# sp-uhh/audio-visual-vad

Measured on AMD Instinct MI355X. Metric: AV frame-pairs/sec (fwd+bwd), higher is better.
Workload: dtype f32; 1 GPU; AV_net fused training step (WaveNet-W0 encoder + ResNet-18 trunk + concat + 2xLSTM1024 + FC, masked BCE, backward, RCCL all-reduce, fused Adam): BASELINE configs[3]/[4] per-GPU shard; per_gpu_frame_pairs=1024, global_frame_pairs=1024, sequences_per_gpu=64, parallelism=dp1, reserved_cus=0, reported_block=median

## Files before the change

audio-visual-vad_amd/csrc/igemm.h:

```cpp
#pragma once
#include "common.h"
#include <type_traits>

namespace igemm {

constexpr int BK = 32;

struct NoCtx {};

struct EpiStore {
  static constexpr bool PLAIN = true;
  float* C;
  long ldc;
  const float* bias;
  int mode;
  int cs = 1;
  double* stat = nullptr;
  __device__ __forceinline__ float* ptr(int m, int n) const { return C + (long)m * ldc + (long)n * cs; }
};
template <class Epi, class = void>
struct HasStat : std::false_type {};
template <class Epi>
struct HasStat<Epi, std::void_t<decltype(Epi::stat)>> : std::true_type {};

// ... 255 lines not shown
  int X, K, relu;
  __device__ __forceinline__ Ctx prep(int) const { return Ctx(); }
  __device__ __forceinline__ typename std::conditional<BUF, void, bool>::type load(const Ctx&, int x, int k0, int kin, float* v) const {
    const int k = k0 + kin;
    const bool ok = k < K && x < X;
    if constexpr (BUF) {
      static_assert(V == 4, "buffer form: 16-byte fetches");
      const f4v t = bload4(brsrc2g(p), ok ? (int)(((unsigned)k * (unsigned)ld + (unsigned)x) * 4u) : BUF_OOB, 0);
      v[0] = t[0]; v[1] = t[1]; v[2] = t[2]; v[3] = t[3];
    } else {
      const long off = ok ? (long)k * ld + x : 0;
      if (V == 4) {
        const float4 t = *reinterpret_cast<const float4*>(p + off);
        v[0] = t.x; v[1] = t.y; v[2] = t.z; v[3] = t.w;
      } else {
        v[0] = p[off];
      }
      return ok;
    }
  }
  __device__ __forceinline__ float post(float v) const { return relu ? fmaxf(v, 0.f) : v; }
};

#ifdef AVVAD_PROF
__device__ unsigned long long g_prof[8];
__device__ unsigned long long g_prof_blk[2 * 2048];
__device__ unsigned long long g_prof_clk[2048];
__device__ unsigned long long g_prof_hw[2048];
#define PROF_T() ((wave == 0) ? __builtin_amdgcn_s_memtime() : 0ull)
#define PROF_ADD(i, v) do { if (t == 0) atomicAdd(&g_prof[i], (unsigned long long)(v)); } while (0)
#else
#define PROF_T() 0ull
#define PROF_ADD(i, v) do { } while (0)
#endif

template <class Op, class = void>
struct HasPost : std::false_type {};
template <class Op>
struct HasPost<Op, std::void_t<decltype(&Op::post)>> : std::true_type {};

template <class Op, class = void>
struct HasPrep2 : std::false_type {};
template <class Op>
struct HasPrep2<Op, std::void_t<decltype(&Op::prep2)>> : std::true_type {};
template <class Op, class = void>
struct PerVec : std::false_type {};
template <class Op>
struct PerVec<Op, std::void_t<decltype(Op::PERVEC)>> : std::integral_constant<bool, Op::PERVEC> {};

template <class Epi, class = void>
struct IsPlain : std::false_type {};
template <class Epi>
struct IsPlain<Epi, std::void_t<decltype(Epi::PLAIN)>> : std::integral_constant<bool, Epi::PLAIN> {};
template <class Epi, class = void>
struct HasFinish : std::false_type {};
template <class Epi>
struct HasFinish<Epi, std::void_t<decltype(&Epi::finish4)>> : std::true_type {};

typedef __bf16 bf16x8 __attribute__((ext_vector_type(8)));
typedef __bf16 bf16x4 __attribute__((ext_vector_type(4)));
typedef float f32x4v __attribute__((ext_vector_type(4)));
constexpr int LDH = 40;

template <class Op, int BX, int NTH>
struct Stage {
  static constexpr int VEC = Op::VEC;
  static constexpr int NV = BX * BK / (NTH * VEC);
  static constexpr int LD = Op::KCONTIG ? BX + 1 : BX + 4;
  static constexpr int NCTX = (Op::KCONTIG || PerVec<Op>::value) ? NV : 1;
  static constexpr int TILE_F32 = BK * LD;
  static constexpr int TILE_BF = BX * LDH / 2;
  __device__ static __forceinline__ void coord(int t, int i, int& xl, int& kl) {
    if (Op::KCONTIG) {
      if (VEC == 4) { kl = (t & 7) * 4; xl = (t >> 3) + (NTH / 8) * i; }
      else { kl = t & 31; xl = (t >> 5) + (NTH / 32) * i; }
    } else {
      if (VEC == 4) { constexpr int Q = BX / 4; xl = (t % Q) * 4; kl = t / Q + (NTH / Q) * i; }
      else { xl = t % BX; kl = t / BX + (NTH / BX) * i; }
    }
  }
  __device__ static __forceinline__ void to_lds(float* S, int t, const float (&st0)[NV][VEC], const Op& op, unsigned okmask) {
    float st[NV][VEC];
#pragma unroll
    for (int i = 0; i < NV; ++i)
#pragma unroll
      for (int j = 0; j < VEC; ++j) {
        float v = st0[i][j];
        if constexpr (HasPost<Op>::value) v = op.post(v);
#ifdef AVVAD_ABL_NOSEL
        st[i][j] = v;
#else
        st[i][j] = ((okmask >> i) & 1u) ? v : 0.f;
#endif
      }
#pragma unroll
    for (int i = 0; i < NV; ++i) {
      int xl, kl;
      coord(t, i, xl, kl);
      if constexpr (Op::KCONTIG) {
#pragma unroll
        for (int j = 0; j < VEC; ++j) S[(kl + j) * LD + xl] = st[i][j];
      } else if constexpr (VEC == 4) {
        *reinterpret_cast<float4*>(S + kl * LD + xl) = make_float4(st[i][0], st[i][1], st[i][2], st[i][3]);
      } else {
        S[kl * LD + xl] = st[i][0];
      }
    }
  }
  __device__ static __forceinline__ void to_lds_bf(__bf16* S, int t, const float (&st0)[NV][VEC], const Op& op, unsigned okmask) {
#pragma unroll
    for (int i = 0; i < NV; ++i) {
// ... 338 lines not shown
#pragma unroll
              for (int r = 0; r < 16; ++r) old[r] = Cb[base + (unsigned)mfma32_row(r, 0) * ld32];
#pragma unroll
              for (int r = 0; r < 16; ++r) Cb[base + (unsigned)mfma32_row(r, 0) * ld32] = old[r] + acc[i][j][r] + bv;
            }
            continue;
          }
        }
#pragma unroll
        for (int r = 0; r < 16; ++r) {
          const int m = mb + mfma32_row(r, lh_e);
          if (m < Mv && n < N) {
            float* p;
            if constexpr (HasSched<Epi>::value) p = Cv + (long)m * E.ldc + n;
            else p = E.ptr(m, n);
            const float v = acc[i][j][r] + bv;
            if (atomic) atomicAdd(p, v);
            else if (E.mode == 0) *p = v;
            else *p += v;
          }
        }
      }
#ifdef AVVAD_PROF
    const unsigned long long tp3 = PROF_T();
    PROF_ADD(0, 1); PROF_ADD(1, tp1 - tp0); PROF_ADD(2, tp2 - tp1); PROF_ADD(3, tbar); PROF_ADD(4, tstage); PROF_ADD(5, tp3 - tp2);
    PROF_ADD(6, kt1 - kt0);
#endif
  }
#ifdef AVVAD_PROF
  if (t == 0 && blockIdx.x < 2048) {
    g_prof_blk[2 * blockIdx.x + 1] = __builtin_amdgcn_s_memrealtime();
    g_prof_clk[blockIdx.x] = __builtin_amdgcn_s_memtime() - g_prof_clk[blockIdx.x];
  }
#endif
}

template <int BM, int BN, class Epi>
__global__ void __launch_bounds__(256)
    fixup(const Epi E, const float* __restrict__ slab, const int M, const int N, const int ktiles, const long G,
          const int full_rounds, const int rem_tiles, const int ntn) {
  constexpr int STRIPS = BM * BN / 256;
  __shared__ float4 part[3][64];
  const int tr = blockIdx.x / STRIPS, strip = blockIdx.x % STRIPS;
  unsigned R = (unsigned)rem_tiles * (unsigned)ktiles, it0 = (unsigned)tr * (unsigned)ktiles, it1 = it0 + (unsigned)ktiles - 1u;
  const unsigned Gu = (unsigned)G;
  if constexpr (HasSched<Epi>::value) {
    R = (unsigned)E.sched.total();
    it0 = (unsigned)E.sched.base(tr);
    it1 = it0 + (unsigned)E.sched.len(tr) - 1u;
  }
  const int ga = (int)(((it0 + 1u) * Gu + R - 1u) / R) - 1, gb = (int)(((it1 + 1u) * Gu + R - 1u) / R) - 1;
  const int lane = threadIdx.x & 63, wave = threadIdx.x >> 6;
  const int e0 = strip * 256 + lane * 4;
  if (gb <= ga) {
    if constexpr (HasFinish<Epi>::value) {
      if (E.active && wave == 0) {
        const unsigned tile_u = (unsigned)full_rounds * Gu + (unsigned)tr;
        const int mu = (int)(tile_u / (unsigned)ntn) * BM + e0 / BN, nu = (int)(tile_u % (unsigned)ntn) * BN + e0 % BN;
        if (epi_live(E, mu, M)) {
          float v[4] = {0.f, 0.f, 0.f, 0.f};
#pragma unroll
          for (int e = 0; e < 4; ++e)
            if (nu + e < N) v[e] = *E.ptr(mu, nu + e);
          E.finish4(mu, nu, v, N);
        }
      }
    }
    return;
  }
  const bool sparse = R < Gu;
  const float* S0 = slab + e0;
  float4 sum = make_float4(0.f, 0.f, 0.f, 0.f);
  for (int g = ga + 1 + wave; g <= gb; g += 16) {
    float4 v[4];
    bool ok[4];
#pragma unroll
    for (int u = 0; u < 4; ++u) {
      const int gu = g + 4 * u;
      ok[u] = gu <= gb && (!sparse || ((unsigned)(gu + 1) * R) / Gu > ((unsigned)gu * R) / Gu);
      v[u] = *reinterpret_cast<const float4*>(S0 + (long)(ok[u] ? gu : ga + 1) * (BM * BN));
    }
#pragma unroll
    for (int u = 0; u < 4; ++u)
      if (ok[u]) { sum.x += v[u].x; sum.y += v[u].y; sum.z += v[u].z; sum.w += v[u].w; }
  }
  if (wave > 0) part[wave - 1][lane] = sum;
  __syncthreads();
  if (wave > 0) return;
#pragma unroll
  for (int w = 0; w < 3; ++w) { const float4 p = part[w][lane]; sum.x += p.x; sum.y += p.y; sum.z += p.z; sum.w += p.w; }
  const unsigned tile = (unsigned)full_rounds * Gu + (unsigned)tr;
  const int m = (int)(tile / (unsigned)ntn) * BM + e0 / BN, n0 = (int)(tile % (unsigned)ntn) * BN + e0 % BN;
  if (!epi_live(E, m, M)) return;
  const float sv[4] = {sum.x, sum.y, sum.z, sum.w};
  if constexpr (HasFinish<Epi>::value) {
    if (E.active) {
      float v[4] = {0.f, 0.f, 0.f, 0.f};
#pragma unroll
      for (int e = 0; e < 4; ++e)
        if (n0 + e < N) v[e] = *E.ptr(m, n0 + e) + sv[e];
      E.finish4(m, n0, v, N);
      return;
    }
  }
#pragma unroll
  for (int e = 0; e < 4; ++e)
    if (n0 + e < N) *E.ptr(m, n0 + e) += sv[e];
}

template <int BM, int BN, class Epi>
__global__ void __launch_bounds__(256)
    fixup1(const Epi E, const float* __restrict__ slab, const int M, const int N, const int ktiles, const long G,
           const int full_rounds, const int rem_tiles, const int ntn) {
  constexpr int STRIPS = BM * BN / 256;
  const int lane = threadIdx.x & 63, wave = threadIdx.x >> 6;
  const int sg = blockIdx.x * 4 + wave;
  const int tr = sg / STRIPS, strip = sg % STRIPS;
  if (tr >= rem_tiles) return;
  unsigned R = (unsigned)rem_tiles * (unsigned)ktiles, it0 = (unsigned)tr * (unsigned)ktiles, it1 = it0 + (unsigned)ktiles - 1u;
  const unsigned Gu = (unsigned)G;
  if constexpr (HasSched<Epi>::value) {
    R = (unsigned)E.sched.total();
    it0 = (unsigned)E.sched.base(tr);
    it1 = it0 + (unsigned)E.sched.len(tr) - 1u;
  }
  const int ga = (int)(((it0 + 1u) * Gu + R - 1u) / R) - 1, gb = (int)(((it1 + 1u) * Gu + R - 1u) / R) - 1;
  const int e0 = strip * 256 + lane * 4;
  const unsigned tile = (unsigned)full_rounds * Gu + (unsigned)tr;
  const int m = (int)(tile / (unsigned)ntn) * BM + e0 / BN, n0 = (int)(tile % (unsigned)ntn) * BN + e0 % BN;
  if (!epi_live(E, m, M)) return;
  float4 sum = make_float4(0.f, 0.f, 0.f, 0.f);
  if (gb > ga) {
    const bool sparse = R < Gu;
    const float* S0 = slab + e0;
    for (int g = ga + 1; g <= gb; g += 4) {
      float4 v[4];
      bool ok[4];
#pragma unroll
      for (int u = 0; u < 4; ++u) {
        const int gu = g + u;
        ok[u] = gu <= gb && (!sparse || ((unsigned)(gu + 1) * R) / Gu > ((unsigned)gu * R) / Gu);
        v[u] = *reinterpret_cast<const float4*>(S0 + (long)(ok[u] ? gu : ga + 1) * (BM * BN));
      }
#pragma unroll
      for (int u = 0; u < 4; ++u)
        if (ok[u]) { sum.x += v[u].x; sum.y += v[u].y; sum.z += v[u].z; sum.w += v[u].w; }
    }
  } else if (!HasFinish<Epi>::value) {
    return;
  }
  const float sv[4] = {sum.x, sum.y, sum.z, sum.w};
  if constexpr (HasFinish<Epi>::value) {
    if (E.active) {
      float v[4] = {0.f, 0.f, 0.f, 0.f};
#pragma unroll
      for (int e = 0; e < 4; ++e)
        if (n0 + e < N) v[e] = *E.ptr(m, n0 + e) + sv[e];
      E.finish4(m, n0, v, N);
      return;
    }
    if (gb <= ga) return;
  }
#pragma unroll
  for (int e = 0; e < 4; ++e)
    if (n0 + e < N) *E.ptr(m, n0 + e) += sv[e];
}

template <int BM, int BN, class Epi = EpiStore>
__global__ void __launch_bounds__(256)
    fixup_tile(const Epi E, const float* __restrict__ slab, const int M, const int N, const int ktiles, const long G,
               const int full_rounds, const int rem_tiles, const int ntn) {
  constexpr int CQ = BN / 4, RG = 256 / CQ, RPT = BM / RG;
  static_assert(RPT % 4 == 0, "four rows in flight per thread");
  __shared__ double red[RG * BN * 2];
  const int tr = blockIdx.x;
  unsigned R = (unsigned)rem_tiles * (unsigned)ktiles, it0 = (unsigned)tr * (unsigned)ktiles, it1 = it0 + (unsigned)ktiles - 1u;
  const unsigned Gu = (unsigned)G;
  if constexpr (HasSched<Epi>::value) {
    R = (unsigned)E.sched.total();
    it0 = (unsigned)E.sched.base(tr);
    it1 = it0 + (unsigned)E.sched.len(tr) - 1u;
  }
  const int ga = (int)(((it0 + 1u) * Gu + R - 1u) / R) - 1, gb = (int)(((it1 + 1u) * Gu + R - 1u) / R) - 1;
  if (gb <= ga) return;
  const bool sparse = R < Gu;
  const unsigned tile = (unsigned)full_rounds * Gu + (unsigned)tr;
  const int tm = (int)(tile / (unsigned)ntn);
  const int m0 = tm * BM, n0 = (int)(tile % (unsigned)ntn) * BN;
  float* Cv = E.C;
  int mrow0 = m0, Mv = M;
  if constexpr (HasSched<Epi>::value) { const auto v = E.view(m0); Cv = v.C; mrow0 = v.row0; Mv = v.M; }
  const int cq = threadIdx.x % CQ, rg = threadIdx.x / CQ;
  const int n = n0 + cq * 4;
  float s4[4] = {0.f, 0.f, 0.f, 0.f}, q4[4] = {0.f, 0.f, 0.f, 0.f};
  if (n < N) {
#pragma unroll 1
    for (int rr = 0; rr < RPT; rr += 4) {
      float4 tot[4];
      bool live[4];
      const float* sp[4];
#pragma unroll
      for (int u = 0; u < 4; ++u) {
        const int row = rg + RG * (rr + u);
        live[u] = mrow0 + row < Mv;
        sp[u] = slab + (long)(live[u] ? row : 0) * BN + cq * 4;
        tot[u] = make_float4(0.f, 0.f, 0.f, 0.f);
      }
      for (int g = ga + 1; g <= gb; ++g) {
        if (sparse && !(((unsigned)(g + 1) * R) / Gu > ((unsigned)g * R) / Gu)) continue;
        float4 v[4];
#pragma unroll
        for (int u = 0; u < 4; ++u) v[u] = *reinterpret_cast<const float4*>(sp[u] + (long)g * (BM * BN));
#pragma unroll
        for (int u = 0; u < 4; ++u) { tot[u].x += v[u].x; tot[u].y += v[u].y; tot[u].z += v[u].z; tot[u].w += v[u].w; }
      }
#pragma unroll
      for (int u = 0; u < 4; ++u) {
        if (!live[u]) continue;
        float4* const cp = reinterpret_cast<float4*>(Cv + (long)(mrow0 + rg + RG * (rr + u)) * E.ldc + n);
        float4 o = *cp;
        o.x += tot[u].x; o.y += tot[u].y; o.z += tot[u].z; o.w += tot[u].w;
        *cp = o;
        s4[0] += o.x; s4[1] += o.y; s4[2] += o.z; s4[3] += o.w;
        q4[0] = fmaf(o.x, o.x, q4[0]); q4[1] = fmaf(o.y, o.y, q4[1]); q4[2] = fmaf(o.z, o.z, q4[2]); q4[3] = fmaf(o.w, o.w, q4[3]);
      }
    }
  }
  if (E.stat == nullptr) return;
#pragma unroll
  for (int e = 0; e < 4; ++e) {
    red[(rg * BN + cq * 4 + e) * 2 + 0] = (double)s4[e];
    red[(rg * BN + cq * 4 + e) * 2 + 1] = (double)q4[e];
  }
  __syncthreads();
  const int c = threadIdx.x;
  if (c < BN && n0 + c < N) {
    double a = 0, b = 0;
#pragma unroll 4
    for (int w = 0; w < RG; ++w) { a += red[(w * BN + c) * 2 + 0]; b += red[(w * BN + c) * 2 + 1]; }
    E.stat[((long)tm * 2 + 0) * N + n0 + c] = a;
    E.stat[((long)tm * 2 + 1) * N + n0 + c] = b;
  }
}

constexpr int NUM_CU = 256;

constexpr size_t SLAB_FLOATS = (size_t)256 * 576 * 64;
static_assert(SLAB_FLOATS >= (size_t)512 * 128 * 128, "one 128x128 tile per persistent worker");

template <int BM, int BN, class AOp, class BOp, class Epi>
static inline int launch(const AOp& a, const BOp& b, const Epi& e_in, int M, int N, int K, int split_k_hint,
                         hipStream_t s, float* slab = nullptr, bool allow_bf16 = true, bool* finished = nullptr) {
  Epi e = e_in;
  if (M <= 0 || N <= 0 || K <= 0) return AVVAD_EINVAL;
  const int ktiles = (K + BK - 1) / BK;
  const long ntiles = (long)cdiv(M, BM) * cdiv(N, BN);
  const long iters = ntiles * ktiles;
  const AvvadTune& tn = avvad_tune();
  const int var = tn.igemm_variant;
  constexpr bool BIG = (BM == 128 && BN == 128);
  constexpr bool TALL = (BM == 256);
  const int variant = TALL ? 3 : (var >= 0 ? var : (BIG ? 2 : 1));
  int per_cu;
  if (variant == 3) per_cu = 2;
  else if (variant == 0) per_cu = BIG ? 2 : (BM * BN >= 128 * 64 ? 3 : 4);
  else if (variant == 1 || !BIG) per_cu = BIG ? 3 : (BM * BN >= 128 * 64 ? 4 : 6);
  else per_cu = 2;
  const int cus = (tn.max_cus > 0 && tn.max_cus < NUM_CU) ? tn.max_cus : NUM_CU;
  long G = (long)cus * per_cu;
  if (G * BM * BN > (long)SLAB_FLOATS) G = (long)(SLAB_FLOATS / ((size_t)BM * BN));
  const bool no_sk = !slab || tn.no_streamk == 1 || tn.no_streamk == 10 + e.mode ||
                     (double)ntiles * ktiles * (double)G >= 4.0e9;
  long full_rounds = ntiles / G, rem = ntiles - full_rounds * G;
  int kchunks = 0;
  if (split_k_hint > 1 && e.mode != 0 && ntiles <= G && tn.kmajor) {
    long best = -1;
    for (int r = 1; r <= 2; ++r) {
      long nc = r * G / ntiles;
      if (nc > ktiles) nc = ktiles;
      if (nc < 1) nc = 1;
      const long rr = (nc * ntiles + G - 1) / G;
      const long cost = rr * ((ktiles + nc - 1) / nc) + rr * 8;
      if (best < 0 || cost < best) { best = cost; kchunks = (int)nc; }
    }
    full_rounds = 0; rem = 0;
    if ((long)kchunks * ntiles < G) G = (long)kchunks * ntiles;
  } else {
    if (no_sk || rem * 10 >= G * 9) {
      if (rem > 0) ++full_rounds;
      rem = 0;
    }
    if (rem > 0 && full_rounds == 0) {
      const long cap = iters / 4 > 0 ? iters / 4 : 1;
      if (G > cap) G = cap;
    }
  }
  const int fr = (int)full_rounds, rt = (int)rem;
  const bool bf = allow_bf16 && tn.bf16;
  bool stat = false;
  if constexpr (std::is_same<Epi, EpiStore>::value) {
    stat = e.stat != nullptr;
    if (stat && (e.cs != 1 || (e.ldc & 3) || (N & 3) || (((uintptr_t)e.C) & 15) || kchunks > 0 || e.bias != nullptr)) return AVVAD_EINVAL;
  }
  if constexpr (HasFinish<Epi>::value) {
    e.active = (rt > 0 && kchunks == 0 && fr == 0 && (long)rt == ntiles) ? 1 : 0;
    if (finished) *finished = e.active != 0;
  } else if (finished) {
    *finished = false;
  }
  const int kflags = tn.stagger ? 1 : 0;
#define AVVAD_IGEMM_LAUNCH(DBV, NTHV)                                                                                       \
  do {                                                                                                                      \
    if (bf)                                                                                                                 \
      hipLaunchKernelGGL((kernel<BM, BN, DBV, NTHV, AOp, BOp, Epi, true>), dim3((int)G), dim3(NTHV), 0, s, a, b, e, M, N, kflags, \
                         ktiles, fr, rt, kchunks, slab);                                                                    \
    else                                                                                                                    \
      hipLaunchKernelGGL((kernel<BM, BN, DBV, NTHV, AOp, BOp, Epi, false>), dim3((int)G), dim3(NTHV), 0, s, a, b, e, M, N, kflags, \
                         ktiles, fr, rt, kchunks, slab);                                                                    \
  } while (0)
  if constexpr (TALL) {
    AVVAD_IGEMM_LAUNCH(false, 512);
  } else {
    if (variant == 0) AVVAD_IGEMM_LAUNCH(true, 256);
    else if (variant == 1 || !BIG) AVVAD_IGEMM_LAUNCH(false, 256);
    else AVVAD_IGEMM_LAUNCH(true, (BIG ? 512 : 256));
  }
#undef AVVAD_IGEMM_LAUNCH
  if (rt > 0 && kchunks == 0 && stat) {
    if constexpr (std::is_same<Epi, EpiStore>::value)
      hipLaunchKernelGGL((fixup_tile<BM, BN>), dim3(rt), dim3(256), 0, s, e, slab, M, N, ktiles, G, fr, rt, cdiv(N, BN));
  } else if (rt > 0 && kchunks == 0) {
    const int deep = tn.no_fixup1 > 1 ? tn.no_fixup1 : 6;
    if ((G + rt - 1) / rt <= deep && tn.no_fixup1 != 1)
      hipLaunchKernelGGL((fixup1<BM, BN, Epi>), dim3(rt * (BM * BN / 1024)), dim3(256), 0, s, e, slab, M, N, ktiles, G, fr, rt, cdiv(N, BN));
    else
      hipLaunchKernelGGL((fixup<BM, BN, Epi>), dim3(rt * (BM * BN / 256)), dim3(256), 0, s, e, slab, M, N, ktiles, G, fr, rt, cdiv(N, BN));
  }
  AVVAD_LAUNCH_CHECK();
  return AVVAD_OK;
}

template <class AOp, class BOp, class Epi>
static inline int launch_cls(const AOp& a, const BOp& b, const Epi& e, int Mp, int N, hipStream_t s, float* slab) {
  constexpr int BM = 128, BN = 128;
  if (Mp <= 0 || N <= 0 || !slab) return AVVAD_EINVAL;
  const AvvadTune& tn = avvad_tune();
  const long ntiles = (long)cdiv(Mp, BM) * cdiv(N, BN);
  const int cus = (tn.max_cus > 0 && tn.max_cus < NUM_CU) ? tn.max_cus : NUM_CU;
  long G = (long)cus * 2;
  if (G * BM * BN > (long)SLAB_FLOATS) G = (long)(SLAB_FLOATS / ((size_t)BM * BN));
  const long R = e.sched.total();
  if (R <= 0 || (double)R * (double)G >= 4.0e9) return AVVAD_EINVAL;
  if (G > R / 4) G = R / 4 > 0 ? R / 4 : 1;
  bool stat = false;
  if constexpr (HasStat<Epi>::value) {
    stat = e.stat != nullptr;
    if (stat && (e.cs != 1 || (e.ldc & 3) || (N & 3) || (((uintptr_t)e.C) & 15) || (e.W & 3))) return AVVAD_EINVAL;
  }
  hipLaunchKernelGGL((kernel<BM, BN, true, 512, AOp, BOp, Epi, false>), dim3((int)G), dim3(512), 0, s, a, b, e, Mp, N,
                     tn.stagger ? 1 : 0, 1, 0, (int)ntiles, 0, slab);
  if (stat) {
    if constexpr (HasStat<Epi>::value)
// ... 14 lines not shown
```

audio-visual-vad_amd/csrc/lstm.hip:

```cpp
#include "gemm_api.h"
#include <stdlib.h>

namespace {


__global__ void add_bias2(const float* __restrict__ a, const float* __restrict__ b, float* __restrict__ o, int n) {
  const int i = blockIdx.x * blockDim.x + threadIdx.x;
  if (i < n) o[i] = a[i] + b[i];
}

__global__ void lstm_gates_fwd(float* __restrict__ G, float* __restrict__ Cs, float* __restrict__ y,
                               const int* __restrict__ lengths, int B, int T, int H, int t) {
  const int idx = blockIdx.x * blockDim.x + threadIdx.x;
  if (idx >= B * H) return;
  const int b = idx / H, j = idx - b * H;
  float* g = G + ((long)b * T + t) * 4 * H;
  const long o = ((long)b * T + t) * H + j;
  if (t >= lengths[b]) {
    g[j] = 0.f; g[H + j] = 0.f; g[2 * H + j] = 0.f; g[3 * H + j] = 0.f;
    Cs[o] = 0.f; y[o] = 0.f;
    return;
  }
  const float ig = sigmoidf_(g[j]), fg = sigmoidf_(g[H + j]), gg = tanhf(g[2 * H + j]), og = sigmoidf_(g[3 * H + j]);
  const float cp = t > 0 ? Cs[o - H] : 0.f;
// ... 195 lines not shown
      }
    }
    if (t + 1 == T) break;
    asm volatile("s_waitcnt vmcnt(0)" ::: "memory");
    __syncthreads();
#ifdef AVVAD_LSTM_PROF
    const unsigned long long s2 = __builtin_amdgcn_s_memrealtime();
#endif
    if (ks == 0 && !give_up) {
      if (lane == 0) __builtin_amdgcn_raw_buffer_store_b32(t, rf, blk * 4, 0, 16);
      int spins = 0;
      for (;;) {
        const i4v f = __builtin_amdgcn_raw_buffer_load_b128(rf, lane * 16, 0, 16);
        const bool mine = (lane * 4 + 0 >= nblk || f[0] >= t) && (lane * 4 + 1 >= nblk || f[1] >= t) &&
                          (lane * 4 + 2 >= nblk || f[2] >= t) && (lane * 4 + 3 >= nblk || f[3] >= t);
        if (__all(mine)) break;
        if (++spins > (1 << 21)) { if (lane == 0) { give_up = 1; sync[1] = 1u; } break; }
      }
    }
    __syncthreads();
#ifdef AVVAD_LSTM_PROF
    const unsigned long long s3 = __builtin_amdgcn_s_memrealtime();
    tA += s1 - s0; tB += s2 - s1; tC += s3 - s2;
#endif
  }
#ifdef AVVAD_LSTM_PROF
  if (threadIdx.x == 0 && blk < 8) {
    unsigned long long* o = reinterpret_cast<unsigned long long*>(sync + 16) + 3 * blk;
    o[0] = tA; o[1] = tB; o[2] = tC;
  }
#endif
}

static int persistent_capacity(int NKp) {
  static int cap[3] = {-1, -1, -1};
  const int i = NKp == 16 ? 0 : (NKp == 8 ? 1 : 2);
  if (cap[i] < 0) {
    int nb = 0, dev = 0, cus = 0;
    hipError_t e = NKp == 16 ? hipOccupancyMaxActiveBlocksPerMultiprocessor(&nb, lstm_persistent_fwd<16>, 256, 0)
                   : NKp == 8 ? hipOccupancyMaxActiveBlocksPerMultiprocessor(&nb, lstm_persistent_fwd<8>, 256, 0)
                              : hipOccupancyMaxActiveBlocksPerMultiprocessor(&nb, lstm_persistent_fwd<4>, 256, 0);
    if (e != hipSuccess || hipGetDevice(&dev) != hipSuccess ||
        hipDeviceGetAttribute(&cus, hipDeviceAttributeMultiprocessorCount, dev) != hipSuccess) { (void)hipGetLastError(); return 0; }
    cap[i] = (nb > 1 ? nb - 1 : nb) * cus;
  }
  return cap[i];
}

__global__ void lstm_persistent_check(const unsigned* __restrict__ sync, float* __restrict__ y, long n) {
  if (sync[1] == 0u) return;
  for (long i = (long)blockIdx.x * blockDim.x + threadIdx.x; i < n; i += (long)gridDim.x * blockDim.x) y[i] = __builtin_nanf("");
}

__global__ void lstm_gates_bwd(float* __restrict__ G, const float* __restrict__ Cs, const float* __restrict__ dy,
                               float* __restrict__ DH, float* __restrict__ DC, const int* __restrict__ lengths, int B,
                               int T, int H, int t) {
  const int idx = blockIdx.x * blockDim.x + threadIdx.x;
  if (idx >= B * H) return;
  const int b = idx / H, j = idx - b * H;
  float* g = G + ((long)b * T + t) * 4 * H;
  const long o = ((long)b * T + t) * H + j;
  const float dhr = DH[idx];
  DH[idx] = 0.f;
  if (t >= lengths[b]) {
    g[j] = 0.f; g[H + j] = 0.f; g[2 * H + j] = 0.f; g[3 * H + j] = 0.f;
    DC[idx] = 0.f;
    return;
  }
  const float ig = g[j], fg = g[H + j], gg = g[2 * H + j], og = g[3 * H + j];
  const float c = Cs[o], cp = t > 0 ? Cs[o - H] : 0.f;
  const float tc = tanhf(c);
  const float dh = dy[o] + dhr;
  const float dc = DC[idx] + dh * og * (1.f - tc * tc);
  g[j] = dc * gg * ig * (1.f - ig);
  g[H + j] = dc * cp * fg * (1.f - fg);
  g[2 * H + j] = dc * ig * (1.f - gg * gg);
  g[3 * H + j] = dh * tc * og * (1.f - og);
  DC[idx] = dc * fg;
}

struct EpiLstmBwd {
  static constexpr bool PLAIN = true;
  float* C;
  long ldc;
  const float* bias;
  int mode;
  int cs;
  int active;
  float* G;
  const float* Cs;
  const float* dy;
  float* DC;
  const int* lengths;
  int T, H, t;
  __device__ __forceinline__ float* ptr(int m, int n) const { return C + (long)m * ldc + n; }
  __device__ __forceinline__ void finish4(int b, int j0, const float (&dhr)[4], int N) const {
    const bool live = t < lengths[b];
    float* g = G + ((long)b * T + t) * 4 * H;
#pragma unroll
    for (int e = 0; e < 4; ++e) {
      const int j = j0 + e;
      if (j >= N) continue;
      const int idx = b * H + j;
      const long o = ((long)b * T + t) * H + j;
      if (!live) {
        g[j] = 0.f; g[H + j] = 0.f; g[2 * H + j] = 0.f; g[3 * H + j] = 0.f;
        DC[idx] = 0.f;
        continue;
      }
      const float ig = g[j], fg = g[H + j], gg = g[2 * H + j], og = g[3 * H + j];
      const float c = Cs[o], cp = t > 0 ? Cs[o - H] : 0.f;
      const float tc = tanhf(c);
      const float dh = dy[o] + dhr[e];
      const float dc = DC[idx] + dh * og * (1.f - tc * tc);
      g[j] = dc * gg * ig * (1.f - ig);
      g[H + j] = dc * cp * fg * (1.f - fg);
      g[2 * H + j] = dc * ig * (1.f - gg * gg);
      g[3 * H + j] = dh * tc * og * (1.f - og);
      DC[idx] = dc * fg;
    }
  }
};

__global__ void shift_time(const float* __restrict__ y, float* __restrict__ ys, int B, int T, int H) {
  const long n = (long)B * T * H;
  for (long i = (long)blockIdx.x * blockDim.x + threadIdx.x; i < n; i += (long)gridDim.x * blockDim.x) {
    const int t = (int)((i / H) % T);
    ys[i] = t > 0 ? y[i - H] : 0.f;
  }
}

__global__ void fill0(float* p, long n) {
  for (long i = (long)blockIdx.x * blockDim.x + threadIdx.x; i < n; i += (long)gridDim.x * blockDim.x) p[i] = 0.f;
}

constexpr int CS_CHUNKS = 64;
__global__ void __launch_bounds__(256)
    colsum_stage1(const float* __restrict__ X, int rows, int cols, float* __restrict__ part) {
  __shared__ float4 sm[4][64];
  const int q = threadIdx.x & 63, rl = threadIdx.x >> 6;
  const int c = (blockIdx.x * 64 + q) * 4;
  const int per = (rows + CS_CHUNKS - 1) / CS_CHUNKS;
  const int r0 = blockIdx.y * per, r1 = min(rows, r0 + per);
  float4 s = make_float4(0.f, 0.f, 0.f, 0.f);
  if (c < cols)
    for (int r = r0 + rl; r < r1; r += 4) {
      const float4 v = *reinterpret_cast<const float4*>(X + (long)r * cols + c);
      s.x += v.x; s.y += v.y; s.z += v.z; s.w += v.w;
    }
  sm[rl][q] = s;
  __syncthreads();
  if (rl == 0 && c < cols) {
    float4 t = sm[0][q];
#pragma unroll
    for (int k = 1; k < 4; ++k) { t.x += sm[k][q].x; t.y += sm[k][q].y; t.z += sm[k][q].z; t.w += sm[k][q].w; }
    *reinterpret_cast<float4*>(part + (long)blockIdx.y * cols + c) = t;
  }
}
__global__ void colsum_stage2(const float* __restrict__ part, int cols, float* __restrict__ out, float* __restrict__ out2) {
  const int c = blockIdx.x * blockDim.x + threadIdx.x;
  if (c >= cols) return;
  float s = 0.f;
  for (int k = 0; k < CS_CHUNKS; ++k) s += part[(long)k * cols + c];
  out[c] += s;
  if (out2) out2[c] += s;
}

struct Ws {
  float *G, *Cs, *bias, *DH, *DC, *Ys, *slab;
  size_t total;
};
static Ws carve(const avvad_lstm_desc* d, float* base) {
  Ws w;
  size_t off = 0;
  auto take = [&](size_t n) { size_t o = off; off += align_up(n, 64); return base ? base + o : (float*)nullptr; };
// ... 38 lines not shown
  const int B = d->B, T = d->T, H = d->H, In = d->In;
  hipLaunchKernelGGL(add_bias2, dim3(cdiv(4 * H, 256)), dim3(256), 0, s, b_ih, b_hh, w.bias, 4 * H);
  int rc;
  avvad_gemm_desc gd = gemm_desc(B * T, 4 * H, In, In, In, 4 * H, 0, 1, 0, 1);
  if ((rc = avvad_gemm_impl(x, w_ih, w.bias, w.G, &gd, s, w.slab))) return rc;
  const int split = pick_split(B, 4 * H, H);
  const int BG = B < 64 ? B : 64;
  const bool fused_step = (B == 16 || B == 32 || (B % 64 == 0 && B <= 65535 * 64)) && (H % (16 * (256 / BG)) == 0) &&
                          !avvad_tune().lstm_no_fused_step && (((uintptr_t)w_hh | (uintptr_t)y) & 15) == 0;
  const int NKp = H / 64;
  const bool persistent = fused_step && !avvad_tune().lstm_no_persistent && B <= 64 && B % 16 == 0 && T > 1 &&
                          (NKp == 16 || NKp == 8 || NKp == 4) && H % 64 == 0 && H / 4 <= 256 &&
                          (long)B * T * H * 4 < (1L << 31);
  if (persistent && H / 4 <= persistent_capacity(NKp)) {
    hipLaunchKernelGGL(lstm_gates_fwd, dim3(cdiv(B * H, 256)), dim3(256), 0, s, w.G, w.Cs, y, d->lengths, B, T, H, 0);
    unsigned* sync = reinterpret_cast<unsigned*>(w.slab);
    if (hipMemsetAsync(sync, 0, 2048, s) != hipSuccess) return AVVAD_ELAUNCH;
    if (NKp == 16) hipLaunchKernelGGL(lstm_persistent_fwd<16>, dim3(H / 4), dim3(256), 0, s, w.G, w.Cs, y, w_hh, d->lengths, B, T, H, sync);
    else if (NKp == 8) hipLaunchKernelGGL(lstm_persistent_fwd<8>, dim3(H / 4), dim3(256), 0, s, w.G, w.Cs, y, w_hh, d->lengths, B, T, H, sync);
    else hipLaunchKernelGGL(lstm_persistent_fwd<4>, dim3(H / 4), dim3(256), 0, s, w.G, w.Cs, y, w_hh, d->lengths, B, T, H, sync);
    hipLaunchKernelGGL(lstm_persistent_check, dim3(64), dim3(256), 0, s, sync, y, (long)B * T * H);
    AVVAD_LAUNCH_CHECK();
    return AVVAD_OK;
  }
  for (int t = 0; t < T; ++t) {
    if (t > 0 && fused_step) {
      if (B >= 128 && H % 16 == 0)
        hipLaunchKernelGGL(lstm_step_fwd_mfma<4>, dim3(H / 16, B / BG), dim3(1024), 0, s, w.G, w.Cs, y, w_hh, d->lengths, B, T, H, t);
      else
        hipLaunchKernelGGL(lstm_step_fwd_mfma<1>, dim3(H / 4, B / BG), dim3(1024), 0, s, w.G, w.Cs, y, w_hh, d->lengths, B, T, H, t);
      continue;
    }
    if (t > 0) {
      avvad_gemm_desc rd = gemm_desc(B, 4 * H, H, T * H, H, T * 4 * H, 0, 1, 1, split);
      if ((rc = avvad_gemm_impl(y + (long)(t - 1) * H, w_hh, nullptr, w.G + (long)t * 4 * H, &rd, s, w.slab))) return rc;
    }
    hipLaunchKernelGGL(lstm_gates_fwd, dim3(cdiv(B * H, 256)), dim3(256), 0, s, w.G, w.Cs, y, d->lengths, B, T, H, t);
  }
  AVVAD_LAUNCH_CHECK();
  return AVVAD_OK;
}

extern "C" int avvad_lstm_layer_bwd(const float* x, const float* w_ih, const float* w_hh, const float* y, const float* dy,
                                    float* dx, float* dw_ih, float* dw_hh, float* db_ih, float* db_hh,
                                    const avvad_lstm_desc* d, void* wsv, size_t ws_bytes, avvad_stream_t sv) {
  AVVAD_ENTER();
  BwdCuCap cu_cap;
  if (!x || !w_ih || !w_hh || !y || !dy || !d || !wsv || !d->lengths || ws_misaligned(wsv)) return AVVAD_EINVAL;
  hipStream_t s = (hipStream_t)sv;
  Ws w = carve(d, (float*)wsv);
  if (ws_bytes < w.total * sizeof(float)) return AVVAD_EWORKSPACE;
  const int B = d->B, T = d->T, H = d->H, In = d->In;
  int rc;
  hipLaunchKernelGGL(fill0, dim3(grid1(B * H)), dim3(256), 0, s, w.DH, (long)B * H);
  hipLaunchKernelGGL(fill0, dim3(grid1(B * H)), dim3(256), 0, s, w.DC, (long)B * H);
  const int split = pick_split(B, H, 4 * H);
  const bool fuse = (B <= 64 || H <= 64) && H % 4 == 0 && ((uintptr_t)w_hh % 16 == 0) && !avvad_tune().lstm_no_fused_step &&
                    (long)B * T * 4 * H < (1L << 29) - 64;
  bool gates_done = false;
  for (int t = T - 1; t >= 0; --t) {
    if (!gates_done)
      hipLaunchKernelGGL(lstm_gates_bwd, dim3(cdiv(B * H, 256)), dim3(256), 0, s, w.G, w.Cs, dy, w.DH, w.DC, d->lengths, B, T,
                         H, t);
    gates_done = false;
    if (t > 0) {
      if (fuse) {
        igemm::RowVec4 a{w.G + (long)t * 4 * H, (long)T * 4 * H, B, 4 * H, 0};
        igemm::ColPlain<4> bop{w_hh, H, H, 4 * H, 0};
        EpiLstmBwd e{w.DH, H, nullptr, 0, 1, 0, w.G, w.Cs, dy, w.DC, d->lengths, T, H, t - 1};
        if ((rc = igemm::launch<64, 64>(a, bop, e, B, H, 4 * H, split, s, w.slab, true, &gates_done))) return rc;
      } else {
        avvad_gemm_desc rd = gemm_desc(B, H, 4 * H, T * 4 * H, H, H, 0, 0, 1, split);
        if ((rc = avvad_gemm_impl(w.G + (long)t * 4 * H, w_hh, nullptr, w.DH, &rd, s, w.slab))) return rc;
      }
    }
  }
  const int R = B * T;
  if (dx) {
    avvad_gemm_desc g1 = gemm_desc(R, In, 4 * H, 4 * H, In, In, 0, 0, 0, 1);
    if ((rc = avvad_gemm_impl(w.G, w_ih, nullptr, dx, &g1, s, w.slab))) return rc;
  }
  if (dw_ih) {
    avvad_gemm_desc g2 = gemm_desc(4 * H, In, R, 4 * H, In, In, 1, 0, 1, pick_split(4 * H, In, R));
    if ((rc = avvad_gemm_impl(w.G, x, nullptr, dw_ih, &g2, s, w.slab))) return rc;
  }
  if (dw_hh) {
    hipLaunchKernelGGL(shift_time, dim3(grid1((long)R * H)), dim3(256), 0, s, y, w.Ys, B, T, H);
    avvad_gemm_desc g3 = gemm_desc(4 * H, H, R, 4 * H, H, H, 1, 0, 1, pick_split(4 * H, H, R));
    if ((rc = avvad_gemm_impl(w.G, w.Ys, nullptr, dw_hh, &g3, s, w.slab))) return rc;
  }
  if (db_ih || db_hh) {
    hipLaunchKernelGGL(colsum_stage1, dim3(cdiv(4 * H, 256), CS_CHUNKS), dim3(256), 0, s, w.G, R, 4 * H, w.slab);
    hipLaunchKernelGGL(colsum_stage2, dim3(cdiv(4 * H, 256)), dim3(256), 0, s, w.slab, 4 * H, db_ih ? db_ih : db_hh,
                       (db_ih && db_hh) ? db_hh : (float*)nullptr);
  }
  AVVAD_LAUNCH_CHECK();
  return AVVAD_OK;
}
```

Before: 60220 frame-pairs/s.

## Add dedicated MFMA split-K LSTM backward step kernel with last-block gate epilogue

Measured after the change: 60310 frame-pairs/s, median of 6. Within noise of the previous version (+0.1%).

```diff
diff --git a/audio-visual-vad_amd/csrc/igemm.h b/audio-visual-vad_amd/csrc/igemm.h
--- a/audio-visual-vad_amd/csrc/igemm.h
+++ b/audio-visual-vad_amd/csrc/igemm.h
@@ -331,11 +331,6 @@
 struct IsPlain : std::false_type {};
 template <class Epi>
 struct IsPlain<Epi, std::void_t<decltype(Epi::PLAIN)>> : std::integral_constant<bool, Epi::PLAIN> {};
-template <class Epi, class = void>
-struct HasFinish : std::false_type {};
-template <class Epi>
-struct HasFinish<Epi, std::void_t<decltype(&Epi::finish4)>> : std::true_type {};
-
 typedef __bf16 bf16x8 __attribute__((ext_vector_type(8)));
 typedef __bf16 bf16x4 __attribute__((ext_vector_type(4)));
 typedef float f32x4v __attribute__((ext_vector_type(4)));
@@ -780,22 +775,7 @@
   const int ga = (int)(((it0 + 1u) * Gu + R - 1u) / R) - 1, gb = (int)(((it1 + 1u) * Gu + R - 1u) / R) - 1;
   const int lane = threadIdx.x & 63, wave = threadIdx.x >> 6;
   const int e0 = strip * 256 + lane * 4;
-  if (gb <= ga) {
-    if constexpr (HasFinish<Epi>::value) {
-      if (E.active && wave == 0) {
-        const unsigned tile_u = (unsigned)full_rounds * Gu + (unsigned)tr;
-        const int mu = (int)(tile_u / (unsigned)ntn) * BM + e0 / BN, nu = (int)(tile_u % (unsigned)ntn) * BN + e0 % BN;
-        if (epi_live(E, mu, M)) {
-          float v[4] = {0.f, 0.f, 0.f, 0.f};
-#pragma unroll
-          for (int e = 0; e < 4; ++e)
-            if (nu + e < N) v[e] = *E.ptr(mu, nu + e);
-          E.finish4(mu, nu, v, N);
-        }
-      }
-    }
-    return;
-  }
+  if (gb <= ga) return;
   const bool sparse = R < Gu;
   const float* S0 = slab + e0;
   float4 sum = make_float4(0.f, 0.f, 0.f, 0.f);
@@ -821,16 +801,6 @@
   const int m = (int)(tile / (unsigned)ntn) * BM + e0 / BN, n0 = (int)(tile % (unsigned)ntn) * BN + e0 % BN;
   if (!epi_live(E, m, M)) return;
   const float sv[4] = {sum.x, sum.y, sum.z, sum.w};
-  if constexpr (HasFinish<Epi>::value) {
-    if (E.active) {
-      float v[4] = {0.f, 0.f, 0.f, 0.f};
-#pragma unroll
-      for (int e = 0; e < 4; ++e)
-        if (n0 + e < N) v[e] = *E.ptr(m, n0 + e) + sv[e];
-      E.finish4(m, n0, v, N);
-      return;
-    }
-  }
 #pragma unroll
   for (int e = 0; e < 4; ++e)
     if (n0 + e < N) *E.ptr(m, n0 + e) += sv[e];
@@ -874,21 +844,10 @@
       for (int u = 0; u < 4; ++u)
         if (ok[u]) { sum.x += v[u].x; sum.y += v[u].y; sum.z += v[u].z; sum.w += v[u].w; }
     }
-  } else if (!HasFinish<Epi>::value) {
+  } else {
     return;
   }
   const float sv[4] = {sum.x, sum.y, sum.z, sum.w};
-  if constexpr (HasFinish<Epi>::value) {
-    if (E.active) {
-      float v[4] = {0.f, 0.f, 0.f, 0.f};
-#pragma unroll
-      for (int e = 0; e < 4; ++e)
-        if (n0 + e < N) v[e] = *E.ptr(m, n0 + e) + sv[e];
-      E.finish4(m, n0, v, N);
-      return;
-    }
-    if (gb <= ga) return;
-  }
 #pragma unroll
   for (int e = 0; e < 4; ++e)
     if (n0 + e < N) *E.ptr(m, n0 + e) += sv[e];
@@ -977,9 +936,8 @@
 static_assert(SLAB_FLOATS >= (size_t)512 * 128 * 128, "one 128x128 tile per persistent worker");
 
 template <int BM, int BN, class AOp, class BOp, class Epi>
-static inline int launch(const AOp& a, const BOp& b, const Epi& e_in, int M, int N, int K, int split_k_hint,
-                         hipStream_t s, float* slab = nullptr, bool allow_bf16 = true, bool* finished = nullptr) {
-  Epi e = e_in;
+static inline int launch(const AOp& a, const BOp& b, const Epi& e, int M, int N, int K, int split_k_hint,
+                         hipStream_t s, float* slab = nullptr, bool allow_bf16 = true) {
   if (M <= 0 || N <= 0 || K <= 0) return AVVAD_EINVAL;
   const int ktiles = (K + BK - 1) / BK;
   const long ntiles = (long)cdiv(M, BM) * cdiv(N, BN);
@@ -1030,12 +988,6 @@
     stat = e.stat != nullptr;
     if (stat && (e.cs != 1 || (e.ldc & 3) || (N & 3) || (((uintptr_t)e.C) & 15) || kchunks > 0 || e.bias != nullptr)) return AVVAD_EINVAL;
   }
-  if constexpr (HasFinish<Epi>::value) {
-    e.active = (rt > 0 && kchunks == 0 && fr == 0 && (long)rt == ntiles) ? 1 : 0;
-    if (finished) *finished = e.active != 0;
-  } else if (finished) {
-    *finished = false;
-  }
   const int kflags = tn.stagger ? 1 : 0;
 #define AVVAD_IGEMM_LAUNCH(DBV, NTHV)                                                                                       \
   do {                                                                                                                      \
diff --git a/audio-visual-vad_amd/csrc/lstm.hip b/audio-visual-vad_amd/csrc/lstm.hip
--- a/audio-visual-vad_amd/csrc/lstm.hip
+++ b/audio-visual-vad_amd/csrc/lstm.hip
@@ -271,75 +271,236 @@
   for (long i = (long)blockIdx.x * blockDim.x + threadIdx.x; i < n; i += (long)gridDim.x * blockDim.x) y[i] = __builtin_nanf("");
 }
 
+__device__ __forceinline__ float gate_bwd_math(float ig, float fg, float gg, float og, float c, float cp, float dyv, float dhr,
+                                               float dcr, float (&d)[4]) {
+  const float tc = tanhf(c);
+  const float dh = dyv + dhr;
+  const float dc = dcr + dh * og * (1.f - tc * tc);
+  d[0] = dc * gg * ig * (1.f - ig);
+  d[1] = dc * cp * fg * (1.f - fg);
+  d[2] = dc * ig * (1.f - gg * gg);
+  d[3] = dh * tc * og * (1.f - og);
+  return dc * fg;
+}
+__device__ __forceinline__ float gate_bwd_dead(float (&d)[4]) {
+  d[0] = 0.f; d[1] = 0.f; d[2] = 0.f; d[3] = 0.f;
+  return 0.f;
+}
+__device__ __forceinline__ float gate_bwd_one(float* __restrict__ g, const float* __restrict__ Cs, const float* __restrict__ dy,
+                                              int H, int j, long o, bool live, bool has_prev, float dhr, float dcr) {
+  float d[4];
+  const float r = live ? gate_bwd_math(g[j], g[H + j], g[2 * H + j], g[3 * H + j], Cs[o], has_prev ? Cs[o - H] : 0.f, dy[o],
+                                       dhr, dcr, d)
+                       : gate_bwd_dead(d);
+  g[j] = d[0]; g[H + j] = d[1]; g[2 * H + j] = d[2]; g[3 * H + j] = d[3];
+  return r;
+}
+
+template <bool FIRST>
 __global__ void lstm_gates_bwd(float* __restrict__ G, const float* __restrict__ Cs, const float* __restrict__ dy,
                                float* __restrict__ DH, float* __restrict__ DC, const int* __restrict__ lengths, int B,
-                               int T, int H, int t) {
+                               int T, int H, int t, unsigned* __restrict__ ctr, int nctr) {
   const int idx = blockIdx.x * blockDim.x + threadIdx.x;
+  if (FIRST && idx < nctr) ctr[idx * 32] = 0u;
   if (idx >= B * H) return;
   const int b = idx / H, j = idx - b * H;
   float* g = G + ((long)b * T + t) * 4 * H;
   const long o = ((long)b * T + t) * H + j;
-  const float dhr = DH[idx];
-  DH[idx] = 0.f;
-  if (t >= lengths[b]) {
-    g[j] = 0.f; g[H + j] = 0.f; g[2 * H + j] = 0.f; g[3 * H + j] = 0.f;
-    DC[idx] = 0.f;
-    return;
-  }
-  const float ig = g[j], fg = g[H + j], gg = g[2 * H + j], og = g[3 * H + j];
-  const float c = Cs[o], cp = t > 0 ? Cs[o - H] : 0.f;
-  const float tc = tanhf(c);
-  const float dh = dy[o] + dhr;
-  const float dc = DC[idx] + dh * og * (1.f - tc * tc);
-  g[j] = dc * gg * ig * (1.f - ig);
-  g[H + j] = dc * cp * fg * (1.f - fg);
-  g[2 * H + j] = dc * ig * (1.f - gg * gg);
-  g[3 * H + j] = dh * tc * og * (1.f - og);
-  DC[idx] = dc * fg;
-}
-
-struct EpiLstmBwd {
-  static constexpr bool PLAIN = true;
-  float* C;
-  long ldc;
-  const float* bias;
-  int mode;
-  int cs;
-  int active;
-  float* G;
-  const float* Cs;
-  const float* dy;
-  float* DC;
-  const int* lengths;
-  int T, H, t;
-  __device__ __forceinline__ float* ptr(int m, int n) const { return C + (long)m * ldc + n; }
-  __device__ __forceinline__ void finish4(int b, int j0, const float (&dhr)[4], int N) const {
-    const bool live = t < lengths[b];
-    float* g = G + ((long)b * T + t) * 4 * H;
+  float dhr = 0.f, dcr = 0.f;
+  if (!FIRST) {
+    dhr = DH[idx];
+    DH[idx] = 0.f;
+    dcr = DC[idx];
+  }
+  DC[idx] = gate_bwd_one(g, Cs, dy, H, j, o, t < lengths[b], t > 0, dhr, dcr);
+}
+
+constexpr int SB_NT = 512;
+constexpr int SB_STEP = 64;
+constexpr int SB_KC = 256;
+constexpr int SB_LDA = SB_KC + 4;
+constexpr int SB_LDT = 64 + 4;
+constexpr int SB_CTR_WORDS = 256 * 32;
+constexpr size_t SB_LDS_BYTES = (size_t)(SB_KC * 64 + 64 * SB_LDA) * sizeof(float);
+__global__ void __launch_bounds__(SB_NT)
+    lstm_step_bwd_mfma(float* __restrict__ G, const float* __restrict__ Cs, const float* __restrict__ dy, float* __restrict__ DC,
+                       const float* __restrict__ w_hh, const int* __restrict__ lengths, int B, int T, int H, int t, int KS,
+                       float* __restrict__ slab, unsigned target) {
+  extern __shared__ __attribute__((aligned(16))) float sb_lds[];
+  __shared__ int is_last;
+  float* const Ws = sb_lds;
+  float* const As = sb_lds + SB_KC * 64;
+  const int tid = threadIdx.x, lane = tid & 63, wave = tid >> 6;
+  const int li = lane & 31, lh = lane >> 5;
+  const int rb = wave & 1, cb = (wave >> 1) & 1, kh = wave >> 2;
+  const int tiles = H >> 6;
+  const int wg = xcd_remap(blockIdx.x, gridDim.x);
+  const int ct = wg % tiles, ks = wg / tiles;
+  const int SL = 4 * H / KS, nstep = SL / SB_STEP;
+  const int k_base = ks * SL, j0 = ct * 64;
+  const __amdgpu_buffer_rsrc_t rG = brsrc2g(G), rW = brsrc2g(w_hh);
+  float* const part = slab + SB_CTR_WORDS;
+  const __amdgpu_buffer_rsrc_t rP = brsrc(part, tiles * KS * 4096 * 4);
+  const int lr = tid >> 4, lc = (tid & 15) * 4;
+  f32x16 acc;
+#pragma unroll
+  for (int r = 0; r < 16; ++r) acc[r] = 0.f;
+  for (int c0 = 0; c0 < nstep; c0 += SB_KC / SB_STEP) {
+    const int nq = min(SB_KC / SB_STEP, nstep - c0);
+    const int kc0 = k_base + c0 * SB_STEP;
+    int oa[8], ow[8];
+#pragma unroll
+    for (int i = 0; i < 8; ++i) {
+      const int q = i >> 1, u = i & 1;
+      const int b = lr + 32 * u;
+      const unsigned a_off = ((unsigned)(b * T + t) * (unsigned)(4 * H) + (unsigned)(kc0 + q * SB_STEP + lc)) * 4u;
+      const unsigned w_off = ((unsigned)(kc0 + i * 32 + lr) * (unsigned)H + (unsigned)(j0 + lc)) * 4u;
+      oa[i] = (q < nq && b < B) ? (int)a_off : BUF_OOB;
+      ow[i] = q < nq ? (int)w_off : BUF_OOB;
+    }
+    f4v wv[8], av[8];
+    __builtin_amdgcn_sched_barrier(0);
+#pragma unroll
+    for (int i = 0; i < 8; ++i) {
+      av[i] = bload4(rG, oa[i], 0);
+      wv[i] = bload4(rW, ow[i], 0);
+      if (i & 1) __syncthreads();
+      __builtin_amdgcn_sched_barrier(0);
+    }
+#pragma unroll
+    for (int q = 0; q < SB_KC / SB_STEP; ++q) {
+      if (q < nq) {
+#pragma unroll
+        for (int u = 0; u < 2; ++u) {
+          *reinterpret_cast<f4v*>(Ws + (q * SB_STEP + u * 32 + lr) * 64 + lc) = wv[2 * q + u];
+          *reinterpret_cast<f4v*>(As + (lr + 32 * u) * SB_LDA + q * SB_STEP + lc) = av[2 * q + u];
+        }
+        __syncthreads();
+#pragma unroll
+        for (int s = 0; s < 4; ++s) {
+          const int kl = q * SB_STEP + kh * 32 + s * 8 + lh * 4;
+          const f4v a = *reinterpret_cast<const f4v*>(As + (rb * 32 + li) * SB_LDA + kl);
+          float bf[4];
+#pragma unroll
+          for (int e = 0; e < 4; ++e) bf[e] = Ws[(kl + e) * 64 + cb * 32 + li];
+#pragma unroll
+          for (int e = 0; e < 4; ++e) acc = mfma32(a[e], bf[e], acc);
+        }
+      }
+    }
+  }
+  const int len[2] = {lengths[lr < B ? lr : 0], lengths[lr + 32 < B ? lr + 32 : 0]};
+  __syncthreads();
+  float* const red = As;
+  float* const tile = As + 4 * 16 * 64;
+  if (kh == 1) {
+#pragma unroll
+    for (int r = 0; r < 16; ++r) red[((wave & 3) * 16 + r) * 64 + lane] = acc[r];
+  }
+  __syncthreads();
+  if (kh == 0) {
+#pragma unroll
+    for (int r = 0; r < 16; ++r)
+      tile[(rb * 32 + mfma32_row(r, lh)) * SB_LDT + cb * 32 + li] = acc[r] + red[((wave & 3) * 16 + r) * 64 + lane];
+  }
+  __syncthreads();
+#pragma unroll
+  for (int u = 0; u < 2; ++u) {
+    const int row = lr + 32 * u;
+    const i4v v = *reinterpret_cast<const i4v*>(tile + row * SB_LDT + lc);
+    __builtin_amdgcn_raw_buffer_store_b128(v, rP, ((ct * KS + ks) * 4096 + row * 64 + lc) * 4, 0, 16);
+  }
+  asm volatile("s_waitcnt vmcnt(0)" ::: "memory");
+  __syncthreads();
+  if (tid == 0) {
+    unsigned* const ctr = reinterpret_cast<unsigned*>(slab) + ct * 32;
+    const unsigned old = __hip_atomic_fetch_add(ctr, 1u, __ATOMIC_RELAXED, __HIP_MEMORY_SCOPE_AGENT);
+    is_last = old + 1u == target;
+  }
+  __syncthreads();
+  if (!is_last) return;
+  const int tp = t - 1;
+  f4v gin[2][4], cv[2], cpv[2], dcv[2];
+  float dyv[2][4];
+  const int cp_back = tp > 0 ? H : 0;
+#pragma unroll
+  for (int u = 0; u < 2; ++u) {
+    const int b = lr + 32 * u, bb = b < B ? b : 0;
+    const float* gp = G + ((long)bb * T + tp) * 4 * H + j0 + lc;
+    const long o = ((long)bb * T + tp) * H + j0 + lc;
+#pragma unroll
+    for (int e = 0; e < 4; ++e) gin[u][e] = *reinterpret_cast<const f4v*>(gp + e * H);
+    cv[u] = *reinterpret_cast<const f4v*>(Cs + o);
+    cpv[u] = *reinterpret_cast<const f4v*>(Cs + o - cp_back);
+    dcv[u] = *reinterpret_cast<const f4v*>(DC + bb * H + j0 + lc);
+#pragma unroll
+    for (int e = 0; e < 4; ++e) dyv[u][e] = dy[o + e];
+  }
+  __builtin_amdgcn_sched_barrier(0);
+  float sum[2][4];
+#pragma unroll
+  for (int u = 0; u < 2; ++u)
+#pragma unroll
+    for (int e = 0; e < 4; ++e) sum[u][e] = 0.f;
+  const int pbase = ct * KS * 4096 + lr * 64 + lc;
+  auto add16 = [&](int s0) {
+    f4v v[16][2];
+#pragma unroll
+    for (int i = 0; i < 16; ++i)
+#pragma unroll
+      for (int u = 0; u < 2; ++u)
+        v[i][u] = __builtin_bit_cast(f4v, __builtin_amdgcn_raw_buffer_load_b128(
+                                              rP, s0 + i < KS ? (pbase + (s0 + i) * 4096 + u * 32 * 64) * 4 : BUF_OOB, 0, 16));
+#pragma unroll
+    for (int i = 0; i < 16; ++i)
+      if (s0 + i < KS) {
+#pragma unroll
+        for (int u = 0; u < 2; ++u)
+#pragma unroll
+          for (int e = 0; e < 4; ++e) sum[u][e] += v[i][u][e];
+      }
+  };
+  add16(0);
+  for (int s0 = 16; s0 < KS; s0 += 16) add16(s0);
+#pragma unroll
+  for (int u = 0; u < 2; ++u) {
+    const int b = lr + 32 * u;
+    if (b >= B) continue;
+    float* gp = G + ((long)b * T + tp) * 4 * H + j0 + lc;
+    f4v o4[4], dcn;
 #pragma unroll
     for (int e = 0; e < 4; ++e) {
-      const int j = j0 + e;
-      if (j >= N) continue;
-      const int idx = b * H + j;
-      const long o = ((long)b * T + t) * H + j;
-      if (!live) {
-        g[j] = 0.f; g[H + j] = 0.f; g[2 * H + j] = 0.f; g[3 * H + j] = 0.f;
-        DC[idx] = 0.f;
-        continue;
-      }
-      const float ig = g[j], fg = g[H + j], gg = g[2 * H + j], og = g[3 * H + j];
-      const float c = Cs[o], cp = t > 0 ? Cs[o - H] : 0.f;
-      const float tc = tanhf(c);
-      const float dh = dy[o] + dhr[e];
-      const float dc = DC[idx] + dh * og * (1.f - tc * tc);
-      g[j] = dc * gg * ig * (1.f - ig);
-      g[H + j] = dc * cp * fg * (1.f - fg);
-      g[2 * H + j] = dc * ig * (1.f - gg * gg);
-      g[3 * H + j] = dh * tc * og * (1.f - og);
-      DC[idx] = dc * fg;
-    }
-  }
-};
+      float d[4];
+      dcn[e] = tp < len[u] ? gate_bwd_math(gin[u][0][e], gin[u][1][e], gin[u][2][e], gin[u][3][e], cv[u][e],
+                                           tp > 0 ? cpv[u][e] : 0.f, dyv[u][e], sum[u][e], dcv[u][e], d)
+                           : gate_bwd_dead(d);
+      o4[0][e] = d[0]; o4[1][e] = d[1]; o4[2][e] = d[2]; o4[3][e] = d[3];
+    }
+#pragma unroll
+    for (int e = 0; e < 4; ++e) *reinterpret_cast<f4v*>(gp + e * H) = o4[e];
+    *reinterpret_cast<f4v*>(DC + b * H + j0 + lc) = dcn;
+  }
+}
+
+static int bwd_step_slices(int H, int cus) {
+  const int tiles = H / 64, steps = 4 * tiles;
+  int ks = 0;
+  for (int k = 1; k <= steps && (long)k * tiles <= cus; ++k)
+    if (steps % k == 0) ks = k;
+  return ks;
+}
+static int device_cus() {
+  static int cus = -1;
+  if (cus < 0) {
+    int dev = 0, n = 0;
+    if (hipGetDevice(&dev) != hipSuccess || hipDeviceGetAttribute(&n, hipDeviceAttributeMultiprocessorCount, dev) != hipSuccess) {
+      (void)hipGetLastError();
+      return 0;
+    }
+    cus = n;
+  }
+  return cus;
+}
 
 __global__ void shift_time(const float* __restrict__ y, float* __restrict__ ys, int B, int T, int H) {
   const long n = (long)B * T * H;
@@ -484,24 +645,29 @@
   if (ws_bytes < w.total * sizeof(float)) return AVVAD_EWORKSPACE;
   const int B = d->B, T = d->T, H = d->H, In = d->In;
   int rc;
-  hipLaunchKernelGGL(fill0, dim3(grid1(B * H)), dim3(256), 0, s, w.DH, (long)B * H);
-  hipLaunchKernelGGL(fill0, dim3(grid1(B * H)), dim3(256), 0, s, w.DC, (long)B * H);
-  const int split = pick_split(B, H, 4 * H);
-  const bool fuse = (B <= 64 || H <= 64) && H % 4 == 0 && ((uintptr_t)w_hh % 16 == 0) && !avvad_tune().lstm_no_fused_step &&
-                    (long)B * T * 4 * H < (1L << 29) - 64;
-  bool gates_done = false;
-  for (int t = T - 1; t >= 0; --t) {
-    if (!gates_done)
-      hipLaunchKernelGGL(lstm_gates_bwd, dim3(cdiv(B * H, 256)), dim3(256), 0, s, w.G, w.Cs, dy, w.DH, w.DC, d->lengths, B, T,
-                         H, t);
-    gates_done = false;
-    if (t > 0) {
-      if (fuse) {
-        igemm::RowVec4 a{w.G + (long)t * 4 * H, (long)T * 4 * H, B, 4 * H, 0};
-        igemm::ColPlain<4> bop{w_hh, H, H, 4 * H, 0};
-        EpiLstmBwd e{w.DH, H, nullptr, 0, 1, 0, w.G, w.Cs, dy, w.DC, d->lengths, T, H, t - 1};
-        if ((rc = igemm::launch<64, 64>(a, bop, e, B, H, 4 * H, split, s, w.slab, true, &gates_done))) return rc;
-      } else {
+  const int cu_dev = device_cus();
+  const int cus = (avvad_tune().max_cus > 0 && avvad_tune().max_cus < cu_dev) ? avvad_tune().max_cus : cu_dev;
+  const int KS = (H % 64 == 0) ? bwd_step_slices(H, cus) : 0;
+  const int tiles = H / 64;
+  const bool step_kernel = B <= 64 && KS > 0 && tiles <= SB_CTR_WORDS / 32 && ((uintptr_t)w_hh % 16 == 0) &&
+                           !avvad_tune().lstm_no_fused_step && (long)B * T * 4 * H < (1L << 29) - 64 &&
+                           (long)4 * H * H < (1L << 29) &&
+                           (size_t)SB_CTR_WORDS + (size_t)tiles * KS * 4096 <= igemm::SLAB_FLOATS;
+  if (step_kernel) {
+    hipLaunchKernelGGL(lstm_gates_bwd<true>, dim3(cdiv(B * H, 256)), dim3(256), 0, s, w.G, w.Cs, dy, w.DH, w.DC, d->lengths, B,
+                       T, H, T - 1, reinterpret_cast<unsigned*>(w.slab), tiles);
+    if (T > 1 && (rc = allow_large_lds<lstm_step_bwd_mfma>(SB_LDS_BYTES, SB_LDS_BYTES))) return rc;
+    for (int t = T - 1; t >= 1; --t)
+      hipLaunchKernelGGL(lstm_step_bwd_mfma, dim3(tiles * KS), dim3(SB_NT), SB_LDS_BYTES, s, w.G, w.Cs, dy, w.DC, w_hh,
+                         d->lengths, B, T, H, t, KS, w.slab, (unsigned)KS * (unsigned)(T - t));
+  } else {
+    hipLaunchKernelGGL(fill0, dim3(grid1(B * H)), dim3(256), 0, s, w.DH, (long)B * H);
+    hipLaunchKernelGGL(fill0, dim3(grid1(B * H)), dim3(256), 0, s, w.DC, (long)B * H);
+    const int split = pick_split(B, H, 4 * H);
+    for (int t = T - 1; t >= 0; --t) {
+      hipLaunchKernelGGL(lstm_gates_bwd<false>, dim3(cdiv(B * H, 256)), dim3(256), 0, s, w.G, w.Cs, dy, w.DH, w.DC, d->lengths,
+                         B, T, H, t, (unsigned*)nullptr, 0);
+      if (t > 0) {
         avvad_gemm_desc rd = gemm_desc(B, H, 4 * H, T * 4 * H, H, H, 0, 0, 1, split);
         if ((rc = avvad_gemm_impl(w.G + (long)t * 4 * H, w_hh, nullptr, w.DH, &rd, s, w.slab))) return rc;
       }
```
